# cgtuebingen/3D-RE-GEN

Hardware: NVIDIA H100
Metric: objects->mesh/sec (256^3 SDF, 50 DiT steps) (higher is better)
Workload: dtype f16

## Files before the change

3d-re-gen_b200/csrc/attn.cu:

```cuda
#include <cuda_fp16.h>
#include <math.h>

#include "r3g_internal.h"
#include "r3g_ptx.cuh"

namespace {

using namespace r3g;

constexpr int kD = 64;
constexpr int kWG = 3;
constexpr int kBQ = 64 * kWG;
constexpr int kBKV = 128;
constexpr int kStg = 3;
constexpr int kQBytes = 64 * kD * 2;
constexpr int kTileBytes = kBKV * kD * 2;
constexpr int kTilesBytes = kQBytes * kWG + 2 * kStg * kTileBytes;
constexpr int kSmemBytes = kTilesBytes + 1024 + 256;
constexpr int kThreads = 128 * kWG + 32;

struct AttnParams {
  __half* o;
  int64_t o_sb, o_sh, o_sl;
  int Lq, Lk;
  float scale_log2;
};

__device__ __forceinline__ float ex2(float x) {
  float y;
  asm("ex2.approx.ftz.f32 %0, %1;" : "=f"(y) : "f"(x));
  return y;
}

__global__ void __launch_bounds__(kThreads, 1)
attention_kernel(const __grid_constant__ CUtensorMap tmap_q, const __grid_constant__ CUtensorMap tmap_k,
                 const __grid_constant__ CUtensorMap tmap_v, const AttnParams p) {
  extern __shared__ uint8_t smem_raw[];
  uint8_t* smem = reinterpret_cast<uint8_t*>((reinterpret_cast<uintptr_t>(smem_raw) + 1023) & ~(uintptr_t)1023);
  uint8_t* sQ = smem;
  uint8_t* sK = sQ + kWG * kQBytes;
  uint8_t* sV = sK + kStg * kTileBytes;
  uint64_t* q_full = reinterpret_cast<uint64_t*>(smem + kTilesBytes);
  uint64_t* k_full = q_full + 1;
  uint64_t* v_full = k_full + kStg;
  uint64_t* k_empty = v_full + kStg;
  uint64_t* v_empty = k_empty + kStg;

  const int warp = threadIdx.x >> 5;
  const int lane = threadIdx.x & 31;
  const int q0 = blockIdx.x * kBQ;
  const int h = blockIdx.y, b = blockIdx.z;
  const int n_kv = (p.Lk + kBKV - 1) / kBKV;

  if (warp == 4 * kWG && lane == 0) {
    tma_prefetch_desc(&tmap_q);
    tma_prefetch_desc(&tmap_k);
    tma_prefetch_desc(&tmap_v);
    mbar_init(q_full, 1);
    for (int s = 0; s < kStg; ++s) {
      mbar_init(&k_full[s], 1);
      mbar_init(&v_full[s], 1);
      mbar_init(&k_empty[s], 128 * kWG);
      mbar_init(&v_empty[s], 128 * kWG);
    }
    fence_barrier_init();
  }
  __syncthreads();
  pdl_wait();

  if (warp == 4 * kWG) {
    if (lane == 0) {
      const int groups = min(kWG, (p.Lq - q0 + 63) / 64);
      mbar_expect_tx(q_full, groups * kQBytes);
      for (int g = 0; g < groups; ++g) tma_load_4d(sQ + g * kQBytes, &tmap_q, q_full, 0, q0 + 64 * g, h, b, kEvictFirst);
      for (int j = 0; j < n_kv; ++j) {
        const int st = j % kStg;
        const uint32_t ph = (j / kStg) & 1;
        mbar_wait(&k_empty[st], ph ^ 1);
        mbar_expect_tx(&k_full[st], kTileBytes);
        tma_load_4d(sK + st * kTileBytes, &tmap_k, &k_full[st], 0, j * kBKV, h, b, kEvictLast);
        mbar_wait(&v_empty[st], ph ^ 1);
        mbar_expect_tx(&v_full[st], kTileBytes);
        tma_load_4d(sV + st * kTileBytes, &tmap_v, &v_full[st], 0, j * kBKV, h, b, kEvictLast);
      }
    }
    return;
  }

  const int wg = warp >> 2;
  const int r0 = (warp & 3) * 16 + (lane >> 2);
  const int c0 = 2 * (lane & 3);
  const uint32_t aq = smem_u32(sQ + wg * kQBytes);
  float o[kD / 2];
#pragma unroll
  for (int i = 0; i < kD / 2; ++i) o[i] = 0.f;
  float m_run[2] = {-INFINITY, -INFINITY}, l_run[2] = {0.f, 0.f};
  mbar_wait(q_full, 0);
  for (int j = 0; j < n_kv; ++j) {
    const int st = j % kStg;
    const uint32_t ph = (j / kStg) & 1;
    float s[kBKV / 2];
    mbar_wait(&k_full[st], ph);
    const uint32_t ak = smem_u32(sK + st * kTileBytes);
    wgmma_fence();
#pragma unroll
    for (int k = 0; k < kD / 16; ++k)
      wgmma_m64n128k16_ss(s, gmma_desc_sw128(aq + k * 32, 1024, 16), gmma_desc_sw128(ak + k * 32, 1024, 16),
                          k ? 1u : 0u);
    wgmma_commit();
    wgmma_wait<0>();
    wgmma_reg_fence<kBKV / 2>(s);
    mbar_arrive(&k_empty[st]);

    const int valid = min(kBKV, p.Lk - j * kBKV);
    if (valid < kBKV) {
#pragma unroll
      for (int i = 0; i < kBKV / 2; ++i)
        if (8 * (i >> 2) + c0 + (i & 1) >= valid) s[i] = -INFINITY;
    }
    float mx[2] = {-INFINITY, -INFINITY};
#pragma unroll
    for (int i = 0; i < kBKV / 2; ++i) mx[(i >> 1) & 1] = fmaxf(mx[(i >> 1) & 1], s[i]);
    float alpha[2];
#pragma unroll
    for (int rr = 0; rr < 2; ++rr) {
      mx[rr] = fmaxf(mx[rr], __shfl_xor_sync(0xffffffffu, mx[rr], 1));
      mx[rr] = fmaxf(mx[rr], __shfl_xor_sync(0xffffffffu, mx[rr], 2));
      const float m_new = fmaxf(m_run[rr], mx[rr] * p.scale_log2);
      alpha[rr] = ex2(m_run[rr] - m_new);
      m_run[rr] = m_new;
      l_run[rr] *= alpha[rr];
    }
#pragma unroll
    for (int i = 0; i < kD / 2; ++i) o[i] *= alpha[(i >> 1) & 1];
    uint32_t pk[kBKV / 16][4];
#pragma unroll
    for (int i = 0; i < kBKV / 2; i += 2) {
      const int rr = (i >> 1) & 1;
      const float e0 = ex2(fmaf(s[i], p.scale_log2, -m_run[rr]));
      const float e1 = ex2(fmaf(s[i + 1], p.scale_log2, -m_run[rr]));
      l_run[rr] += e0 + e1;
      pk[i >> 3][(i >> 1) & 3] = pack_half2(e0, e1);
    }
    mbar_wait(&v_full[st], ph);
    const uint32_t av = smem_u32(sV + st * kTileBytes);
    wgmma_fence();
#pragma unroll
    for (int k = 0; k < kBKV / 16; ++k) wgmma_m64n64k16_rs_tb(o, pk[k], gmma_desc_sw128(av + k * 2048, 1024, 1024), 1u);
    wgmma_commit();
    wgmma_wait<0>();
    wgmma_reg_fence<kD / 2>(o);
    mbar_arrive(&v_empty[st]);
  }

  float inv_l[2];
#pragma unroll
  for (int rr = 0; rr < 2; ++rr) {
    float l = l_run[rr];
    l += __shfl_xor_sync(0xffffffffu, l, 1);
    l += __shfl_xor_sync(0xffffffffu, l, 2);
    inv_l[rr] = 1.f / l;
  }
#pragma unroll
  for (int rr = 0; rr < 2; ++rr) {
    const int qrow = q0 + wg * 64 + r0 + 8 * rr;
    if (qrow >= p.Lq) continue;
    __half* op = p.o + (int64_t)b * p.o_sb + (int64_t)h * p.o_sh + (int64_t)qrow * p.o_sl;
#pragma unroll
    for (int i = 2 * rr; i < kD / 2; i += 4)
      *reinterpret_cast<uint32_t*>(op + 8 * (i >> 2) + c0) = pack_half2(o[i] * inv_l[rr], o[i + 1] * inv_l[rr]);
  }
}

int make_qkv_map(r3g_ctx* ctx, CUtensorMap* m, const void* base, int64_t sb, int64_t sh, int64_t sl, int B, int H,
                 int L, int box_rows) {
  const uint64_t dims[4] = {(uint64_t)kD, (uint64_t)L, (uint64_t)H, (uint64_t)B};
  const uint64_t strides[4] = {2, (uint64_t)sl * 2, (uint64_t)sh * 2, (uint64_t)sb * 2};
  const uint32_t box[4] = {(uint32_t)kD, (uint32_t)box_rows, 1, 1};
  return r3g_make_tmap_f16(ctx, m, base, 4, dims, strides, box);
}

}

extern "C" int r3g_attention(r3g_ctx* ctx, const r3g_attention_args* a, void* stream) {
  r3g_device_guard guard(ctx);
  if (!ctx || !ctx->encode_tiled)
    return r3g_fail(ctx, R3G_E_CUDA, "attention: no CUDA device (there is no CPU fallback)");
  if (!a || !a->q || !a->k || !a->v || !a->o) return r3g_fail(ctx, R3G_E_INVALID, "attention: null argument");
  if (a->B < 1 || a->H < 1 || a->Lq < 1 || a->Lk < 1) return r3g_fail(ctx, R3G_E_INVALID, "attention: empty shape");
  if (a->o_sl % 8 || a->o_sh % 8 || a->o_sb % 8 || ((uintptr_t)a->o) % 16)
    return r3g_fail(ctx, R3G_E_INVALID, "attention: output strides must be multiples of 8 halfs");
  CUtensorMap mq, mk, mv;
  int rc;
  if ((rc = make_qkv_map(ctx, &mq, a->q, a->q_sb, a->q_sh, a->q_sl, a->B, a->H, a->Lq, 64))) return rc;
  if ((rc = make_qkv_map(ctx, &mk, a->k, a->k_sb, a->k_sh, a->k_sl, a->B, a->H, a->Lk, kBKV))) return rc;
  if ((rc = make_qkv_map(ctx, &mv, a->v, a->v_sb, a->v_sh, a->v_sl, a->B, a->H, a->Lk, kBKV))) return rc;
  AttnParams p;
  p.o = (__half*)a->o;
  p.o_sb = a->o_sb; p.o_sh = a->o_sh; p.o_sl = a->o_sl;
  p.Lq = a->Lq; p.Lk = a->Lk;
  p.scale_log2 = a->scale * 1.4426950408889634f;
  if (!(ctx->attr_done & R3G_ATTR_ATTENTION)) {
    R3G_CUDA_OK(ctx, cudaFuncSetAttribute(attention_kernel, cudaFuncAttributeMaxDynamicSharedMemorySize, kSmemBytes));
    R3G_CUDA_OK(ctx, cudaFuncSetAttribute(attention_kernel, cudaFuncAttributePreferredSharedMemoryCarveout, 100));
    ctx->attr_done |= R3G_ATTR_ATTENTION;
  }
  dim3 grid((a->Lq + kBQ - 1) / kBQ, a->H, a->B);
  R3G_CUDA_OK(ctx, r3g_launch_pdl(ctx, attention_kernel, grid, dim3(kThreads), kSmemBytes, (cudaStream_t)stream, mq, mk, mv, p));
  R3G_LAUNCH_OK(ctx);
  return R3G_OK;
}
```

3d-re-gen_b200/csrc/r3g_ptx.cuh:

```cuda
#pragma once
#include <cuda.h>
#include <cuda_fp16.h>
#include <cuda_runtime.h>
#include <stdint.h>

namespace r3g {

__device__ __forceinline__ uint32_t smem_u32(const void* p) {
  return static_cast<uint32_t>(__cvta_generic_to_shared(p));
}

__device__ __forceinline__ bool elect_one() {
  uint32_t pred = 0;
  asm volatile(
      "{\n\t.reg .pred P;\n\t"
      "elect.sync _|P, 0xffffffff;\n\t"
      "selp.u32 %0, 1, 0, P;\n\t}\n"
      : "=r"(pred));
  return pred != 0;
}

__device__ __forceinline__ void mbar_init(uint64_t* bar, uint32_t count) {
  asm volatile("mbarrier.init.shared::cta.b64 [%0], %1;\n" ::"r"(smem_u32(bar)), "r"(count));
}
__device__ __forceinline__ void pdl_wait() { asm volatile("griddepcontrol.wait;" ::: "memory"); }
__device__ __forceinline__ void pdl_trigger() { asm volatile("griddepcontrol.launch_dependents;" ::: "memory"); }

__device__ __forceinline__ void fence_barrier_init() {
  asm volatile("fence.mbarrier_init.release.cluster;\n" ::: "memory");
}
__device__ __forceinline__ void mbar_expect_tx(uint64_t* bar, uint32_t bytes) {
  asm volatile("mbarrier.arrive.expect_tx.shared::cta.b64 _, [%0], %1;\n" ::"r"(smem_u32(bar)), "r"(bytes)
               : "memory");
}
__device__ __forceinline__ void mbar_arrive(uint64_t* bar) {
  asm volatile("mbarrier.arrive.shared::cta.b64 _, [%0];\n" ::"r"(smem_u32(bar)) : "memory");
}
constexpr uint32_t kMbarSuspendHint = 0x989680u;
__device__ __forceinline__ bool mbar_try_wait(uint64_t* bar, uint32_t parity) {
  uint32_t ok;
  asm volatile(
      "{\n\t.reg .pred P;\n\t"
      "mbarrier.try_wait.parity.shared::cta.b64 P, [%1], %2, %3;\n\t"
      "selp.u32 %0, 1, 0, P;\n\t}\n"
      : "=r"(ok)
      : "r"(smem_u32(bar)), "r"(parity), "r"(kMbarSuspendHint)
      : "memory");
  return ok != 0;
}
__device__ __forceinline__ void mbar_wait(uint64_t* bar, uint32_t parity) {
  while (!mbar_try_wait(bar, parity)) {
  }
}

__device__ __forceinline__ void fence_proxy_async_smem() {
  asm volatile("fence.proxy.async.shared::cta;\n" ::: "memory");
}

__device__ __forceinline__ void named_bar_sync(uint32_t id, uint32_t count) {
  asm volatile("bar.sync %0, %1;\n" ::"r"(id), "r"(count) : "memory");
}

__device__ __forceinline__ void tma_prefetch_desc(const CUtensorMap* m) {
  asm volatile("prefetch.tensormap [%0];\n" ::"l"(reinterpret_cast<uint64_t>(m)) : "memory");
}
constexpr uint64_t kEvictNormal = 0x1000000000000000ull;
constexpr uint64_t kEvictFirst = 0x12F0000000000000ull;
constexpr uint64_t kEvictLast = 0x14F0000000000000ull;

__device__ __forceinline__ void tma_load_2d(void* smem_dst, const CUtensorMap* m, uint64_t* bar, int c0, int c1,
                                            uint64_t hint = kEvictNormal) {
  asm volatile(
      "cp.async.bulk.tensor.2d.shared::cluster.global.mbarrier::complete_tx::bytes.L2::cache_hint"
      " [%0], [%1, {%3, %4}], [%2], %5;\n" ::"r"(smem_u32(smem_dst)),
      "l"(reinterpret_cast<uint64_t>(m)), "r"(smem_u32(bar)), "r"(c0), "r"(c1), "l"(hint)
      : "memory");
}
__device__ __forceinline__ void tma_load_3d(void* smem_dst, const CUtensorMap* m, uint64_t* bar, int c0, int c1,
                                            int c2, uint64_t hint = kEvictNormal) {
  asm volatile(
      "cp.async.bulk.tensor.3d.shared::cluster.global.mbarrier::complete_tx::bytes.L2::cache_hint"
      " [%0], [%1, {%3, %4, %5}], [%2], %6;\n" ::"r"(smem_u32(smem_dst)),
      "l"(reinterpret_cast<uint64_t>(m)), "r"(smem_u32(bar)), "r"(c0), "r"(c1), "r"(c2), "l"(hint)
      : "memory");
}
__device__ __forceinline__ void tma_load_4d(void* smem_dst, const CUtensorMap* m, uint64_t* bar, int c0, int c1,
                                            int c2, int c3, uint64_t hint = kEvictNormal) {
  asm volatile(
      "cp.async.bulk.tensor.4d.shared::cluster.global.mbarrier::complete_tx::bytes.L2::cache_hint"
      " [%0], [%1, {%3, %4, %5, %6}], [%2], %7;\n" ::"r"(smem_u32(smem_dst)),
      "l"(reinterpret_cast<uint64_t>(m)), "r"(smem_u32(bar)), "r"(c0), "r"(c1), "r"(c2), "r"(c3), "l"(hint)
      : "memory");
}

__device__ __forceinline__ void wgmma_fence() { asm volatile("wgmma.fence.sync.aligned;\n" ::: "memory"); }
__device__ __forceinline__ void wgmma_commit() { asm volatile("wgmma.commit_group.sync.aligned;\n" ::: "memory"); }
template <int N>
__device__ __forceinline__ void wgmma_wait() {
  asm volatile("wgmma.wait_group.sync.aligned %0;\n" ::"n"(N) : "memory");
}
template <int N>
__device__ __forceinline__ void wgmma_reg_fence(float* d) {
#pragma unroll
  for (int i = 0; i < N; ++i) asm volatile("" : "+f"(d[i])::"memory");
}
__device__ __forceinline__ void wgmma_m64n128k16_ss(float* d, uint64_t desc_a, uint64_t desc_b, uint32_t accumulate) {
  asm volatile(
      "{\n\t.reg .pred p;\n\t"
      "setp.ne.b32 p, %66, 0;\n\t"
      "wgmma.mma_async.sync.aligned.m64n128k16.f32.f16.f16 "
      "{%0, %1, %2, %3, %4, %5, %6, %7, %8, %9, %10, %11, %12, %13, %14, %15, %16, %17, %18, %19, %20, %21, %22, %23, %24, %25, %26, %27, %28, %29, %30, %31, %32, %33, %34, %35, %36, %37, %38, %39, %40, %41, %42, %43, %44, %45, %46, %47, %48, %49, %50, %51, %52, %53, %54, %55, %56, %57, %58, %59, %60, %61, %62, %63}, "
      "%64, %65, p, 1, 1, 0, 0;\n\t}\n"
      : "+f"(d[0]), "+f"(d[1]), "+f"(d[2]), "+f"(d[3]), "+f"(d[4]), "+f"(d[5]), "+f"(d[6]), "+f"(d[7]), "+f"(d[8]), "+f"(d[9]), "+f"(d[10]), "+f"(d[11]), "+f"(d[12]), "+f"(d[13]), "+f"(d[14]), "+f"(d[15]), "+f"(d[16]), "+f"(d[17]), "+f"(d[18]), "+f"(d[19]), "+f"(d[20]), "+f"(d[21]), "+f"(d[22]), "+f"(d[23]), "+f"(d[24]), "+f"(d[25]), "+f"(d[26]), "+f"(d[27]), "+f"(d[28]), "+f"(d[29]), "+f"(d[30]), "+f"(d[31]), "+f"(d[32]), "+f"(d[33]), "+f"(d[34]), "+f"(d[35]), "+f"(d[36]), "+f"(d[37]), "+f"(d[38]), "+f"(d[39]), "+f"(d[40]), "+f"(d[41]), "+f"(d[42]), "+f"(d[43]), "+f"(d[44]), "+f"(d[45]), "+f"(d[46]), "+f"(d[47]), "+f"(d[48]), "+f"(d[49]), "+f"(d[50]), "+f"(d[51]), "+f"(d[52]), "+f"(d[53]), "+f"(d[54]), "+f"(d[55]), "+f"(d[56]), "+f"(d[57]), "+f"(d[58]), "+f"(d[59]), "+f"(d[60]), "+f"(d[61]), "+f"(d[62]), "+f"(d[63])
      : "l"(desc_a), "l"(desc_b), "r"(accumulate));
}
__device__ __forceinline__ void wgmma_m64n256k16_ss(float* d, uint64_t desc_a, uint64_t desc_b, uint32_t accumulate) {
  asm volatile(
      "{\n\t.reg .pred p;\n\t"
      "setp.ne.b32 p, %130, 0;\n\t"
      "wgmma.mma_async.sync.aligned.m64n256k16.f32.f16.f16 "
      "{%0, %1, %2, %3, %4, %5, %6, %7, %8, %9, %10, %11, %12, %13, %14, %15, %16, %17, %18, %19, %20, %21, %22, %23, %24, %25, %26, %27, %28, %29, %30, %31, %32, %33, %34, %35, %36, %37, %38, %39, %40, %41, %42, %43, %44, %45, %46, %47, %48, %49, %50, %51, %52, %53, %54, %55, %56, %57, %58, %59, %60, %61, %62, %63, %64, %65, %66, %67, %68, %69, %70, %71, %72, %73, %74, %75, %76, %77, %78, %79, %80, %81, %82, %83, %84, %85, %86, %87, %88, %89, %90, %91, %92, %93, %94, %95, %96, %97, %98, %99, %100, %101, %102, %103, %104, %105, %106, %107, %108, %109, %110, %111, %112, %113, %114, %115, %116, %117, %118, %119, %120, %121, %122, %123, %124, %125, %126, %127}, "
      "%128, %129, p, 1, 1, 0, 0;\n\t}\n"
      : "+f"(d[0]), "+f"(d[1]), "+f"(d[2]), "+f"(d[3]), "+f"(d[4]), "+f"(d[5]), "+f"(d[6]), "+f"(d[7]), "+f"(d[8]), "+f"(d[9]), "+f"(d[10]), "+f"(d[11]), "+f"(d[12]), "+f"(d[13]), "+f"(d[14]), "+f"(d[15]), "+f"(d[16]), "+f"(d[17]), "+f"(d[18]), "+f"(d[19]), "+f"(d[20]), "+f"(d[21]), "+f"(d[22]), "+f"(d[23]), "+f"(d[24]), "+f"(d[25]), "+f"(d[26]), "+f"(d[27]), "+f"(d[28]), "+f"(d[29]), "+f"(d[30]), "+f"(d[31]), "+f"(d[32]), "+f"(d[33]), "+f"(d[34]), "+f"(d[35]), "+f"(d[36]), "+f"(d[37]), "+f"(d[38]), "+f"(d[39]), "+f"(d[40]), "+f"(d[41]), "+f"(d[42]), "+f"(d[43]), "+f"(d[44]), "+f"(d[45]), "+f"(d[46]), "+f"(d[47]), "+f"(d[48]), "+f"(d[49]), "+f"(d[50]), "+f"(d[51]), "+f"(d[52]), "+f"(d[53]), "+f"(d[54]), "+f"(d[55]), "+f"(d[56]), "+f"(d[57]), "+f"(d[58]), "+f"(d[59]), "+f"(d[60]), "+f"(d[61]), "+f"(d[62]), "+f"(d[63]), "+f"(d[64]), "+f"(d[65]), "+f"(d[66]), "+f"(d[67]), "+f"(d[68]), "+f"(d[69]), "+f"(d[70]), "+f"(d[71]), "+f"(d[72]), "+f"(d[73]), "+f"(d[74]), "+f"(d[75]), "+f"(d[76]), "+f"(d[77]), "+f"(d[78]), "+f"(d[79]), "+f"(d[80]), "+f"(d[81]), "+f"(d[82]), "+f"(d[83]), "+f"(d[84]), "+f"(d[85]), "+f"(d[86]), "+f"(d[87]), "+f"(d[88]), "+f"(d[89]), "+f"(d[90]), "+f"(d[91]), "+f"(d[92]), "+f"(d[93]), "+f"(d[94]), "+f"(d[95]), "+f"(d[96]), "+f"(d[97]), "+f"(d[98]), "+f"(d[99]), "+f"(d[100]), "+f"(d[101]), "+f"(d[102]), "+f"(d[103]), "+f"(d[104]), "+f"(d[105]), "+f"(d[106]), "+f"(d[107]), "+f"(d[108]), "+f"(d[109]), "+f"(d[110]), "+f"(d[111]), "+f"(d[112]), "+f"(d[113]), "+f"(d[114]), "+f"(d[115]), "+f"(d[116]), "+f"(d[117]), "+f"(d[118]), "+f"(d[119]), "+f"(d[120]), "+f"(d[121]), "+f"(d[122]), "+f"(d[123]), "+f"(d[124]), "+f"(d[125]), "+f"(d[126]), "+f"(d[127])
      : "l"(desc_a), "l"(desc_b), "r"(accumulate));
}
__device__ __forceinline__ void wgmma_m64n64k16_rs_tb(float* d, const uint32_t* a, uint64_t desc_b, uint32_t accumulate) {
  asm volatile(
      "{\n\t.reg .pred p;\n\t"
      "setp.ne.b32 p, %37, 0;\n\t"
      "wgmma.mma_async.sync.aligned.m64n64k16.f32.f16.f16 "
      "{%0, %1, %2, %3, %4, %5, %6, %7, %8, %9, %10, %11, %12, %13, %14, %15, %16, %17, %18, %19, %20, %21, %22, %23, %24, %25, %26, %27, %28, %29, %30, %31}, "
      "{%32, %33, %34, %35}, %36, p, 1, 1, 1;\n\t}\n"
      : "+f"(d[0]), "+f"(d[1]), "+f"(d[2]), "+f"(d[3]), "+f"(d[4]), "+f"(d[5]), "+f"(d[6]), "+f"(d[7]), "+f"(d[8]), "+f"(d[9]), "+f"(d[10]), "+f"(d[11]), "+f"(d[12]), "+f"(d[13]), "+f"(d[14]), "+f"(d[15]), "+f"(d[16]), "+f"(d[17]), "+f"(d[18]), "+f"(d[19]), "+f"(d[20]), "+f"(d[21]), "+f"(d[22]), "+f"(d[23]), "+f"(d[24]), "+f"(d[25]), "+f"(d[26]), "+f"(d[27]), "+f"(d[28]), "+f"(d[29]), "+f"(d[30]), "+f"(d[31])
      : "r"(a[0]), "r"(a[1]), "r"(a[2]), "r"(a[3]), "l"(desc_b), "r"(accumulate));
}
__device__ __forceinline__ uint64_t f2_pack(float lo, float hi) {
  uint64_t r;
  asm("mov.b64 %0, {%1, %2};" : "=l"(r) : "f"(lo), "f"(hi));
  return r;
}
__device__ __forceinline__ void f2_unpack(uint64_t v, float& lo, float& hi) {
  asm("mov.b64 {%0, %1}, %2;" : "=f"(lo), "=f"(hi) : "l"(v));
}
__device__ __forceinline__ uint64_t f2_fma(uint64_t a, uint64_t b, uint64_t c) {
  float a0, a1, b0, b1, c0, c1;
  f2_unpack(a, a0, a1); f2_unpack(b, b0, b1); f2_unpack(c, c0, c1);
  return f2_pack(__fmaf_rn(a0, b0, c0), __fmaf_rn(a1, b1, c1));
}
__device__ __forceinline__ uint64_t f2_add(uint64_t a, uint64_t b) {
  float a0, a1, b0, b1;
  f2_unpack(a, a0, a1); f2_unpack(b, b0, b1);
  return f2_pack(__fadd_rn(a0, b0), __fadd_rn(a1, b1));
}
__device__ __forceinline__ uint64_t f2_mul(uint64_t a, uint64_t b) {
  float a0, a1, b0, b1;
  f2_unpack(a, a0, a1); f2_unpack(b, b0, b1);
  return f2_pack(__fmul_rn(a0, b0), __fmul_rn(a1, b1));
}

__device__ __forceinline__ uint64_t gmma_desc_sw128(uint32_t saddr, uint32_t sbo_bytes, uint32_t lbo_bytes) {
  uint64_t d = 0;
  d |= (uint64_t)((saddr & 0x3FFFF) >> 4);
  d |= (uint64_t)((lbo_bytes >> 4) & 0x3FFF) << 16;
  d |= (uint64_t)((sbo_bytes >> 4) & 0x3FFF) << 32;
  d |= (uint64_t)1 << 62;
  return d;
}

__device__ __forceinline__ uint32_t pack_half2(float a, float b) {
  __half2 h = __floats2half2_rn(a, b);
  return *reinterpret_cast<uint32_t*>(&h);
}

}
```

Measured before the change: 0.2704.

## Make attention kernel persistent with intra-warpgroup QK/PV overlap and ping-pong scheduling

Turns the attention kernel into a persistent kernel that loops over (q-tile, head, batch) tiles with a grid sized to the SM count, and double-buffers Q so the next tile's Q load overlaps the current one. Consumer warpgroups now issue the next QK GEMM before the current PV GEMM and run softmax while PV is in flight, FA3-style. Named barriers pass an MMA turn between warpgroups so tensor-core issue is serialized in a ping-pong. Producer warps give up registers through setmaxnreg so the consumers can hold more. The cost is more complex synchronization, extra shared memory for Q, and a full warpgroup assigned to the producer.

New measurement: 0.2766 (median of 6 runs). 1.02x the previous value.

```diff
diff --git a/3d-re-gen_b200/csrc/attn.cu b/3d-re-gen_b200/csrc/attn.cu
--- a/3d-re-gen_b200/csrc/attn.cu
+++ b/3d-re-gen_b200/csrc/attn.cu
@@ -13,17 +13,42 @@
 constexpr int kBQ = 64 * kWG;
 constexpr int kBKV = 128;
 constexpr int kStg = 3;
+constexpr int kQStg = 2;
 constexpr int kQBytes = 64 * kD * 2;
 constexpr int kTileBytes = kBKV * kD * 2;
-constexpr int kTilesBytes = kQBytes * kWG + 2 * kStg * kTileBytes;
+constexpr int kTilesBytes = kQStg * kWG * kQBytes + 2 * kStg * kTileBytes;
 constexpr int kSmemBytes = kTilesBytes + 1024 + 256;
-constexpr int kThreads = 128 * kWG + 32;
+constexpr int kThreads = 128 * (kWG + 1);
+constexpr int kProducerRegs = 24;
+constexpr int kConsumerRegs = 160;
+static_assert(128 * (kWG * kConsumerRegs + kProducerRegs) <= 65536, "register file");
 
 struct AttnParams {
   __half* o;
   int64_t o_sb, o_sh, o_sl;
   int Lq, Lk;
+  int H, n_qt, n_tiles;
   float scale_log2;
+};
+
+struct Tile {
+  int q0, h, b;
+};
+__device__ __forceinline__ Tile tile_at(int t, const AttnParams& p) {
+  const int bh = t / p.n_qt;
+  return {(t - bh * p.n_qt) * kBQ, bh % p.H, bh / p.H};
+}
+
+template <int kDepth>
+struct RingPos {
+  int st = 0;
+  uint32_t ph = 0;
+  __device__ __forceinline__ void next() {
+    if (++st == kDepth) {
+      st = 0;
+      ph ^= 1;
+    }
+  }
 };
 
 __device__ __forceinline__ float ex2(float x) {
@@ -31,6 +56,66 @@
   asm("ex2.approx.ftz.f32 %0, %1;" : "=f"(y) : "f"(x));
   return y;
 }
+
+__device__ __forceinline__ void reg_fence_a(uint32_t (&a)[kBKV / 16][4]) {
+#pragma unroll
+  for (int k = 0; k < kBKV / 16; ++k)
+#pragma unroll
+    for (int i = 0; i < 4; ++i) asm volatile("" : "+r"(a[k][i])::"memory");
+}
+
+__device__ __forceinline__ void issue_qk(float (&s)[kBKV / 2], uint32_t aq, uint32_t ak) {
+  wgmma_fence();
+#pragma unroll
+  for (int k = 0; k < kD / 16; ++k)
+    wgmma_m64n128k16_ss(s, gmma_desc_sw128(aq + k * 32, 1024, 16), gmma_desc_sw128(ak + k * 32, 1024, 16), k ? 1u : 0u);
+  wgmma_commit();
+}
+
+__device__ __forceinline__ void issue_pv(float (&o)[kD / 2], const uint32_t (&pk)[kBKV / 16][4], uint32_t av) {
+  wgmma_fence();
+#pragma unroll
+  for (int k = 0; k < kBKV / 16; ++k) wgmma_m64n64k16_rs_tb(o, pk[k], gmma_desc_sw128(av + k * 2048, 1024, 1024), 1u);
+  wgmma_commit();
+}
+
+__device__ __forceinline__ void softmax_tile(float (&s)[kBKV / 2], int valid, int c0, float scale_log2,
+                                             float (&m_run)[2], float (&l_run)[2], float (&alpha)[2]) {
+  if (valid < kBKV) {
+#pragma unroll
+    for (int i = 0; i < kBKV / 2; ++i)
+      if (8 * (i >> 2) + c0 + (i & 1) >= valid) s[i] = -INFINITY;
+  }
+  float mx[2] = {-INFINITY, -INFINITY};
+#pragma unroll
+  for (int i = 0; i < kBKV / 2; ++i) mx[(i >> 1) & 1] = fmaxf(mx[(i >> 1) & 1], s[i]);
+#pragma unroll
+  for (int rr = 0; rr < 2; ++rr) {
+    mx[rr] = fmaxf(mx[rr], __shfl_xor_sync(0xffffffffu, mx[rr], 1));
+    mx[rr] = fmaxf(mx[rr], __shfl_xor_sync(0xffffffffu, mx[rr], 2));
+    const float m_new = fmaxf(m_run[rr], mx[rr] * scale_log2);
+    alpha[rr] = ex2(m_run[rr] - m_new);
+    m_run[rr] = m_new;
+    l_run[rr] *= alpha[rr];
+  }
+#pragma unroll
+  for (int i = 0; i < kBKV / 2; i += 2) {
+    const int rr = (i >> 1) & 1;
+    const float e0 = ex2(fmaf(s[i], scale_log2, -m_run[rr]));
+    const float e1 = ex2(fmaf(s[i + 1], scale_log2, -m_run[rr]));
+    l_run[rr] += e0 + e1;
+    s[i] = e0;
+    s[i + 1] = e1;
+  }
+}
+
+__device__ __forceinline__ void pack_p(const float (&s)[kBKV / 2], uint32_t (&pk)[kBKV / 16][4]) {
+#pragma unroll
+  for (int i = 0; i < kBKV / 2; i += 2) pk[i >> 3][(i >> 1) & 3] = pack_half2(s[i], s[i + 1]);
+}
+
+__device__ __forceinline__ void mma_turn_wait() { named_bar_sync(1 + (threadIdx.x >> 7), 256); }
+__device__ __forceinline__ void mma_turn_pass() { named_bar_arrive(1 + ((threadIdx.x >> 7) + 1) % kWG, 256); }
 
 __global__ void __launch_bounds__(kThreads, 1)
 attention_kernel(const __grid_constant__ CUtensorMap tmap_q, const __grid_constant__ CUtensorMap tmap_k,
@@ -38,25 +123,27 @@
   extern __shared__ uint8_t smem_raw[];
   uint8_t* smem = reinterpret_cast<uint8_t*>((reinterpret_cast<uintptr_t>(smem_raw) + 1023) & ~(uintptr_t)1023);
   uint8_t* sQ = smem;
-  uint8_t* sK = sQ + kWG * kQBytes;
+  uint8_t* sK = sQ + kQStg * kWG * kQBytes;
   uint8_t* sV = sK + kStg * kTileBytes;
   uint64_t* q_full = reinterpret_cast<uint64_t*>(smem + kTilesBytes);
-  uint64_t* k_full = q_full + 1;
+  uint64_t* q_empty = q_full + kQStg;
+  uint64_t* k_full = q_empty + kQStg;
   uint64_t* v_full = k_full + kStg;
   uint64_t* k_empty = v_full + kStg;
   uint64_t* v_empty = k_empty + kStg;
 
   const int warp = threadIdx.x >> 5;
   const int lane = threadIdx.x & 31;
-  const int q0 = blockIdx.x * kBQ;
-  const int h = blockIdx.y, b = blockIdx.z;
   const int n_kv = (p.Lk + kBKV - 1) / kBKV;
 
   if (warp == 4 * kWG && lane == 0) {
     tma_prefetch_desc(&tmap_q);
     tma_prefetch_desc(&tmap_k);
     tma_prefetch_desc(&tmap_v);
-    mbar_init(q_full, 1);
+    for (int s = 0; s < kQStg; ++s) {
+      mbar_init(&q_full[s], 1);
+      mbar_init(&q_empty[s], 128 * kWG);
+    }
     for (int s = 0; s < kStg; ++s) {
       mbar_init(&k_full[s], 1);
       mbar_init(&v_full[s], 1);
@@ -68,108 +155,135 @@
   __syncthreads();
   pdl_wait();
 
-  if (warp == 4 * kWG) {
-    if (lane == 0) {
-      const int groups = min(kWG, (p.Lq - q0 + 63) / 64);
-      mbar_expect_tx(q_full, groups * kQBytes);
-      for (int g = 0; g < groups; ++g) tma_load_4d(sQ + g * kQBytes, &tmap_q, q_full, 0, q0 + 64 * g, h, b, kEvictFirst);
-      for (int j = 0; j < n_kv; ++j) {
-        const int st = j % kStg;
-        const uint32_t ph = (j / kStg) & 1;
-        mbar_wait(&k_empty[st], ph ^ 1);
-        mbar_expect_tx(&k_full[st], kTileBytes);
-        tma_load_4d(sK + st * kTileBytes, &tmap_k, &k_full[st], 0, j * kBKV, h, b, kEvictLast);
-        mbar_wait(&v_empty[st], ph ^ 1);
-        mbar_expect_tx(&v_full[st], kTileBytes);
-        tma_load_4d(sV + st * kTileBytes, &tmap_v, &v_full[st], 0, j * kBKV, h, b, kEvictLast);
+  if (warp >= 4 * kWG) {
+    setmaxnreg_dec<kProducerRegs>();
+    if (warp == 4 * kWG && lane == 0) {
+      RingPos<kQStg> qs;
+      RingPos<kStg> kv;
+      for (int t = blockIdx.x; t < p.n_tiles; t += gridDim.x) {
+        const Tile tl = tile_at(t, p);
+        const int groups = min(kWG, (p.Lq - tl.q0 + 63) / 64);
+        mbar_wait(&q_empty[qs.st], qs.ph ^ 1);
+        mbar_expect_tx(&q_full[qs.st], groups * kQBytes);
+        for (int g = 0; g < groups; ++g)
+          tma_load_4d(sQ + (qs.st * kWG + g) * kQBytes, &tmap_q, &q_full[qs.st], 0, tl.q0 + 64 * g, tl.h, tl.b,
+                      kEvictFirst);
+        qs.next();
+        for (int j = 0; j < n_kv; ++j, kv.next()) {
+          mbar_wait(&k_empty[kv.st], kv.ph ^ 1);
+          mbar_expect_tx(&k_full[kv.st], kTileBytes);
+          tma_load_4d(sK + kv.st * kTileBytes, &tmap_k, &k_full[kv.st], 0, j * kBKV, tl.h, tl.b, kEvictLast);
+          mbar_wait(&v_empty[kv.st], kv.ph ^ 1);
+          mbar_expect_tx(&v_full[kv.st], kTileBytes);
+          tma_load_4d(sV + kv.st * kTileBytes, &tmap_v, &v_full[kv.st], 0, j * kBKV, tl.h, tl.b, kEvictLast);
+        }
       }
     }
     return;
   }
 
+  setmaxnreg_inc<kConsumerRegs>();
   const int wg = warp >> 2;
-  const int r0 = (warp & 3) * 16 + (lane >> 2);
   const int c0 = 2 * (lane & 3);
-  const uint32_t aq = smem_u32(sQ + wg * kQBytes);
-  float o[kD / 2];
-#pragma unroll
-  for (int i = 0; i < kD / 2; ++i) o[i] = 0.f;
-  float m_run[2] = {-INFINITY, -INFINITY}, l_run[2] = {0.f, 0.f};
-  mbar_wait(q_full, 0);
-  for (int j = 0; j < n_kv; ++j) {
-    const int st = j % kStg;
-    const uint32_t ph = (j / kStg) & 1;
+  RingPos<kQStg> qs;
+  RingPos<kStg> kv;
+  if (wg == kWG - 1) mma_turn_pass();
+  for (int t = blockIdx.x; t < p.n_tiles; t += gridDim.x) {
+    mbar_wait(&q_full[qs.st], qs.ph);
+    if (tile_at(t, p).q0 + 64 * wg >= p.Lq) {
+      RingPos<kStg> kk = kv;
+      for (int j = 0; j <= n_kv; ++j) {
+        mma_turn_wait();
+        mma_turn_pass();
+        if (j < n_kv) {
+          mbar_wait(&k_full[kk.st], kk.ph);
+          mbar_arrive(&k_empty[kk.st]);
+          kk.next();
+        }
+        if (j > 0) {
+          mbar_wait(&v_full[kv.st], kv.ph);
+          mbar_arrive(&v_empty[kv.st]);
+          kv.next();
+        }
+      }
+      mbar_arrive(&q_empty[qs.st]);
+      qs.next();
+      continue;
+    }
+    const uint32_t aq = smem_u32(sQ + (qs.st * kWG + wg) * kQBytes);
+    float o[kD / 2];
+#pragma unroll
+    for (int i = 0; i < kD / 2; ++i) o[i] = 0.f;
+    float m_run[2] = {-INFINITY, -INFINITY}, l_run[2] = {0.f, 0.f}, alpha[2];
     float s[kBKV / 2];
-    mbar_wait(&k_full[st], ph);
-    const uint32_t ak = smem_u32(sK + st * kTileBytes);
-    wgmma_fence();
-#pragma unroll
-    for (int k = 0; k < kD / 16; ++k)
-      wgmma_m64n128k16_ss(s, gmma_desc_sw128(aq + k * 32, 1024, 16), gmma_desc_sw128(ak + k * 32, 1024, 16),
-                          k ? 1u : 0u);
-    wgmma_commit();
+    uint32_t pk[kBKV / 16][4];
+
+    mma_turn_wait();
+    mbar_wait(&k_full[kv.st], kv.ph);
+    issue_qk(s, aq, smem_u32(sK + kv.st * kTileBytes));
+    mma_turn_pass();
     wgmma_wait<0>();
     wgmma_reg_fence<kBKV / 2>(s);
-    mbar_arrive(&k_empty[st]);
-
-    const int valid = min(kBKV, p.Lk - j * kBKV);
-    if (valid < kBKV) {
-#pragma unroll
-      for (int i = 0; i < kBKV / 2; ++i)
-        if (8 * (i >> 2) + c0 + (i & 1) >= valid) s[i] = -INFINITY;
-    }
-    float mx[2] = {-INFINITY, -INFINITY};
-#pragma unroll
-    for (int i = 0; i < kBKV / 2; ++i) mx[(i >> 1) & 1] = fmaxf(mx[(i >> 1) & 1], s[i]);
-    float alpha[2];
-#pragma unroll
-    for (int rr = 0; rr < 2; ++rr) {
-      mx[rr] = fmaxf(mx[rr], __shfl_xor_sync(0xffffffffu, mx[rr], 1));
-      mx[rr] = fmaxf(mx[rr], __shfl_xor_sync(0xffffffffu, mx[rr], 2));
-      const float m_new = fmaxf(m_run[rr], mx[rr] * p.scale_log2);
-      alpha[rr] = ex2(m_run[rr] - m_new);
-      m_run[rr] = m_new;
-      l_run[rr] *= alpha[rr];
-    }
-#pragma unroll
-    for (int i = 0; i < kD / 2; ++i) o[i] *= alpha[(i >> 1) & 1];
-    uint32_t pk[kBKV / 16][4];
-#pragma unroll
-    for (int i = 0; i < kBKV / 2; i += 2) {
-      const int rr = (i >> 1) & 1;
-      const float e0 = ex2(fmaf(s[i], p.scale_log2, -m_run[rr]));
-      const float e1 = ex2(fmaf(s[i + 1], p.scale_log2, -m_run[rr]));
-      l_run[rr] += e0 + e1;
-      pk[i >> 3][(i >> 1) & 3] = pack_half2(e0, e1);
-    }
-    mbar_wait(&v_full[st], ph);
-    const uint32_t av = smem_u32(sV + st * kTileBytes);
-    wgmma_fence();
-#pragma unroll
-    for (int k = 0; k < kBKV / 16; ++k) wgmma_m64n64k16_rs_tb(o, pk[k], gmma_desc_sw128(av + k * 2048, 1024, 1024), 1u);
-    wgmma_commit();
+    mbar_arrive(&k_empty[kv.st]);
+    softmax_tile(s, min(kBKV, p.Lk), c0, p.scale_log2, m_run, l_run, alpha);
+    for (int j = 0;; ++j) {
+      wgmma_wait<0>();
+      wgmma_reg_fence<kD / 2>(o);
+      reg_fence_a(pk);
+      if (j > 0) {
+        mbar_arrive(&v_empty[kv.st]);
+        kv.next();
+      }
+#pragma unroll
+      for (int i = 0; i < kD / 2; ++i) o[i] *= alpha[(i >> 1) & 1];
+      pack_p(s, pk);
+      if (j + 1 == n_kv) break;
+      RingPos<kStg> nx = kv;
+      nx.next();
+      mma_turn_wait();
+      mbar_wait(&k_full[nx.st], nx.ph);
+      issue_qk(s, aq, smem_u32(sK + nx.st * kTileBytes));
+      mbar_wait(&v_full[kv.st], kv.ph);
+      issue_pv(o, pk, smem_u32(sV + kv.st * kTileBytes));
+      mma_turn_pass();
+      wgmma_wait<1>();
+      wgmma_reg_fence<kBKV / 2>(s);
+      mbar_arrive(&k_empty[nx.st]);
+      softmax_tile(s, min(kBKV, p.Lk - (j + 1) * kBKV), c0, p.scale_log2, m_run, l_run, alpha);
+    }
+    mma_turn_wait();
+    mbar_wait(&v_full[kv.st], kv.ph);
+    issue_pv(o, pk, smem_u32(sV + kv.st * kTileBytes));
+    mma_turn_pass();
     wgmma_wait<0>();
     wgmma_reg_fence<kD / 2>(o);
-    mbar_arrive(&v_empty[st]);
-  }
-
-  float inv_l[2];
-#pragma unroll
-  for (int rr = 0; rr < 2; ++rr) {
-    float l = l_run[rr];
-    l += __shfl_xor_sync(0xffffffffu, l, 1);
-    l += __shfl_xor_sync(0xffffffffu, l, 2);
-    inv_l[rr] = 1.f / l;
-  }
-#pragma unroll
-  for (int rr = 0; rr < 2; ++rr) {
-    const int qrow = q0 + wg * 64 + r0 + 8 * rr;
-    if (qrow >= p.Lq) continue;
-    __half* op = p.o + (int64_t)b * p.o_sb + (int64_t)h * p.o_sh + (int64_t)qrow * p.o_sl;
-#pragma unroll
-    for (int i = 2 * rr; i < kD / 2; i += 4)
-      *reinterpret_cast<uint32_t*>(op + 8 * (i >> 2) + c0) = pack_half2(o[i] * inv_l[rr], o[i + 1] * inv_l[rr]);
-  }
+    reg_fence_a(pk);
+    mbar_arrive(&v_empty[kv.st]);
+    kv.next();
+    mbar_arrive(&q_empty[qs.st]);
+    qs.next();
+
+    float inv_l[2];
+#pragma unroll
+    for (int rr = 0; rr < 2; ++rr) {
+      float l = l_run[rr];
+      l += __shfl_xor_sync(0xffffffffu, l, 1);
+      l += __shfl_xor_sync(0xffffffffu, l, 2);
+      inv_l[rr] = 1.f / l;
+    }
+    const Tile tl = tile_at(t, p);
+    const int r0 = ((threadIdx.x >> 1) & 48) + ((threadIdx.x & 31) >> 2);
+#pragma unroll
+    for (int rr = 0; rr < 2; ++rr) {
+      const int qrow = tl.q0 + wg * 64 + r0 + 8 * rr;
+      if (qrow >= p.Lq) continue;
+      __half* op = p.o + (int64_t)tl.b * p.o_sb + (int64_t)tl.h * p.o_sh + (int64_t)qrow * p.o_sl;
+#pragma unroll
+      for (int i = 2 * rr; i < kD / 2; i += 4)
+        *reinterpret_cast<uint32_t*>(op + 8 * (i >> 2) + c0) = pack_half2(o[i] * inv_l[rr], o[i + 1] * inv_l[rr]);
+    }
+  }
+  if (wg == 0) mma_turn_wait();
 }
 
 int make_qkv_map(r3g_ctx* ctx, CUtensorMap* m, const void* base, int64_t sb, int64_t sh, int64_t sl, int B, int H,
@@ -199,13 +313,18 @@
   p.o = (__half*)a->o;
   p.o_sb = a->o_sb; p.o_sh = a->o_sh; p.o_sl = a->o_sl;
   p.Lq = a->Lq; p.Lk = a->Lk;
+  p.H = a->H;
+  p.n_qt = (a->Lq + kBQ - 1) / kBQ;
+  const int64_t tiles = (int64_t)p.n_qt * a->H * a->B;
+  if (tiles > INT32_MAX) return r3g_fail(ctx, R3G_E_INVALID, "attention: too many query tiles");
+  p.n_tiles = (int)tiles;
   p.scale_log2 = a->scale * 1.4426950408889634f;
   if (!(ctx->attr_done & R3G_ATTR_ATTENTION)) {
     R3G_CUDA_OK(ctx, cudaFuncSetAttribute(attention_kernel, cudaFuncAttributeMaxDynamicSharedMemorySize, kSmemBytes));
     R3G_CUDA_OK(ctx, cudaFuncSetAttribute(attention_kernel, cudaFuncAttributePreferredSharedMemoryCarveout, 100));
     ctx->attr_done |= R3G_ATTR_ATTENTION;
   }
-  dim3 grid((a->Lq + kBQ - 1) / kBQ, a->H, a->B);
+  const dim3 grid((unsigned)(tiles < ctx->num_sms ? tiles : ctx->num_sms));
   R3G_CUDA_OK(ctx, r3g_launch_pdl(ctx, attention_kernel, grid, dim3(kThreads), kSmemBytes, (cudaStream_t)stream, mq, mk, mv, p));
   R3G_LAUNCH_OK(ctx);
   return R3G_OK;
diff --git a/3d-re-gen_b200/csrc/r3g_ptx.cuh b/3d-re-gen_b200/csrc/r3g_ptx.cuh
--- a/3d-re-gen_b200/csrc/r3g_ptx.cuh
+++ b/3d-re-gen_b200/csrc/r3g_ptx.cuh
@@ -53,12 +53,20 @@
   }
 }
 
+template <int N>
+__device__ __forceinline__ void setmaxnreg_dec() { asm volatile("setmaxnreg.dec.sync.aligned.u32 %0;\n" ::"n"(N)); }
+template <int N>
+__device__ __forceinline__ void setmaxnreg_inc() { asm volatile("setmaxnreg.inc.sync.aligned.u32 %0;\n" ::"n"(N)); }
+
 __device__ __forceinline__ void fence_proxy_async_smem() {
   asm volatile("fence.proxy.async.shared::cta;\n" ::: "memory");
 }
 
 __device__ __forceinline__ void named_bar_sync(uint32_t id, uint32_t count) {
   asm volatile("bar.sync %0, %1;\n" ::"r"(id), "r"(count) : "memory");
+}
+__device__ __forceinline__ void named_bar_arrive(uint32_t id, uint32_t count) {
+  asm volatile("bar.arrive %0, %1;\n" ::"r"(id), "r"(count) : "memory");
 }
 
 __device__ __forceinline__ void tma_prefetch_desc(const CUtensorMap* m) {
```

## Software-pipeline attention QK and PV wgmma with producer/consumer register reallocation

Applied to the files above, without the earlier changes.

Restructures the attention consumer loop so the QK^T wgmma for tile j is issued together with the PV wgmma for tile j-1. Softmax on the new scores then runs while the PV matmul is in flight, hiding tensor-core latency behind exp work. The producer is widened to a full warpgroup that calls setmaxnreg to give up registers, so consumer warpgroups can raise their limit to 160. Empty barriers now count only the active warpgroups, and idle ones exit early. The extra live registers (scores plus the packed P from the previous tile) add spill risk, and the ordering of waits and barriers is harder to get right.

New measurement: 0.2682 before, 0.2702 after (median of 6 runs). Within noise of the previous version (+0.7%).

```diff
diff --git a/3d-re-gen_b200/csrc/attn.cu b/3d-re-gen_b200/csrc/attn.cu
--- a/3d-re-gen_b200/csrc/attn.cu
+++ b/3d-re-gen_b200/csrc/attn.cu
@@ -17,7 +17,9 @@
 constexpr int kTileBytes = kBKV * kD * 2;
 constexpr int kTilesBytes = kQBytes * kWG + 2 * kStg * kTileBytes;
 constexpr int kSmemBytes = kTilesBytes + 1024 + 256;
-constexpr int kThreads = 128 * kWG + 32;
+constexpr int kThreads = 128 * (kWG + 1);
+constexpr uint32_t kProducerRegs = 24, kConsumerRegs = 160;
+static_assert(128 * kProducerRegs + 128 * kWG * kConsumerRegs <= 65536, "register split exceeds the register file");
 
 struct AttnParams {
   __half* o;
@@ -30,6 +32,87 @@
   float y;
   asm("ex2.approx.ftz.f32 %0, %1;" : "=f"(y) : "f"(x));
   return y;
+}
+
+__device__ __forceinline__ void issue_qk(float (&s)[kBKV / 2], uint32_t aq, uint32_t ak) {
+#pragma unroll
+  for (int k = 0; k < kD / 16; ++k)
+    wgmma_m64n128k16_ss(s, gmma_desc_sw128(aq + k * 32, 1024, 16), gmma_desc_sw128(ak + k * 32, 1024, 16), k ? 1u : 0u);
+}
+
+__device__ __forceinline__ void issue_pv(float (&o)[kD / 2], const uint32_t (&pk)[kBKV / 16][4], uint32_t av) {
+#pragma unroll
+  for (int k = 0; k < kBKV / 16; ++k) wgmma_m64n64k16_rs_tb(o, pk[k], gmma_desc_sw128(av + k * 2048, 1024, 1024), 1u);
+}
+
+template <bool kMask>
+__device__ __forceinline__ void softmax_tile(float (&s)[kBKV / 2], float (&m_run)[2], float (&l_run)[2],
+                                             float (&alpha)[2], int valid, int c0, float scale_log2) {
+  if (kMask) {
+#pragma unroll
+    for (int i = 0; i < kBKV / 2; ++i) s[i] = 8 * (i >> 2) + c0 + (i & 1) >= valid ? -INFINITY : s[i];
+  }
+  float mx[2] = {-INFINITY, -INFINITY};
+#pragma unroll
+  for (int i = 0; i < kBKV / 2; ++i) mx[(i >> 1) & 1] = fmaxf(mx[(i >> 1) & 1], s[i]);
+#pragma unroll
+  for (int rr = 0; rr < 2; ++rr) {
+    mx[rr] = fmaxf(mx[rr], __shfl_xor_sync(0xffffffffu, mx[rr], 1));
+    mx[rr] = fmaxf(mx[rr], __shfl_xor_sync(0xffffffffu, mx[rr], 2));
+    const float m_new = fmaxf(m_run[rr], mx[rr] * scale_log2);
+    alpha[rr] = ex2(m_run[rr] - m_new);
+    m_run[rr] = m_new;
+    l_run[rr] *= alpha[rr];
+  }
+#pragma unroll
+  for (int i = 0; i < kBKV / 2; i += 2) {
+    const int rr = (i >> 1) & 1;
+    const float e0 = ex2(fmaf(s[i], scale_log2, -m_run[rr]));
+    const float e1 = ex2(fmaf(s[i + 1], scale_log2, -m_run[rr]));
+    l_run[rr] += e0 + e1;
+    s[i] = e0;
+    s[i + 1] = e1;
+  }
+}
+
+__device__ __forceinline__ void pack_p(uint32_t (&pk)[kBKV / 16][4], const float (&s)[kBKV / 2]) {
+#pragma unroll
+  for (int i = 0; i < kBKV / 2; i += 2) pk[i >> 3][(i >> 1) & 3] = pack_half2(s[i], s[i + 1]);
+}
+
+__device__ __forceinline__ void pin_before_wait(uint32_t sink, float v) {
+  asm volatile("st.shared.f32 [%0], %1;\n" ::"r"(sink), "f"(v) : "memory");
+}
+
+template <bool kMask>
+__device__ __forceinline__ void pipelined_tile(int j, int valid, float (&o)[kD / 2], uint32_t (&pk)[kBKV / 16][4],
+                                               float (&m_run)[2], float (&l_run)[2], float (&alpha)[2], uint32_t aq,
+                                               int c0, uint8_t* sK, uint8_t* sV, uint64_t* k_full, uint64_t* v_full,
+                                               uint64_t* k_empty, uint64_t* v_empty, uint32_t sink,
+                                               float scale_log2) {
+  const int st = j % kStg, pst = (j - 1) % kStg;
+  const uint32_t ph = (j / kStg) & 1, pph = ((j - 1) / kStg) & 1;
+  float s[kBKV / 2];
+  mbar_wait(&k_full[st], ph);
+  wgmma_fence();
+  issue_qk(s, aq, smem_u32(sK + st * kTileBytes));
+  wgmma_commit();
+#pragma unroll
+  for (int i = 0; i < kD / 2; ++i) o[i] *= alpha[(i >> 1) & 1];
+  mbar_wait(&v_full[pst], pph);
+  wgmma_fence();
+  issue_pv(o, pk, smem_u32(sV + pst * kTileBytes));
+  wgmma_commit();
+  wgmma_wait<1>();
+  wgmma_reg_fence<kBKV / 2>(s);
+  mbar_arrive(&k_empty[st]);
+  softmax_tile<kMask>(s, m_run, l_run, alpha, valid, c0, scale_log2);
+  pin_before_wait(sink, l_run[0] + l_run[1]);
+  wgmma_wait<0>();
+  wgmma_reg_fence<kD / 2>(o);
+  wgmma_reg_fence_u32<kBKV / 8>(&pk[0][0]);
+  mbar_arrive(&v_empty[pst]);
+  pack_p(pk, s);
 }
 
 __global__ void __launch_bounds__(kThreads, 1)
@@ -45,12 +128,14 @@
   uint64_t* v_full = k_full + kStg;
   uint64_t* k_empty = v_full + kStg;
   uint64_t* v_empty = k_empty + kStg;
+  const uint32_t sink = smem_u32(v_empty + kStg);
 
   const int warp = threadIdx.x >> 5;
   const int lane = threadIdx.x & 31;
   const int q0 = blockIdx.x * kBQ;
   const int h = blockIdx.y, b = blockIdx.z;
   const int n_kv = (p.Lk + kBKV - 1) / kBKV;
+  const int groups = min(kWG, (p.Lq - q0 + 63) / 64);
 
   if (warp == 4 * kWG && lane == 0) {
     tma_prefetch_desc(&tmap_q);
@@ -60,17 +145,17 @@
     for (int s = 0; s < kStg; ++s) {
       mbar_init(&k_full[s], 1);
       mbar_init(&v_full[s], 1);
-      mbar_init(&k_empty[s], 128 * kWG);
-      mbar_init(&v_empty[s], 128 * kWG);
+      mbar_init(&k_empty[s], 128 * groups);
+      mbar_init(&v_empty[s], 128 * groups);
     }
     fence_barrier_init();
   }
   __syncthreads();
   pdl_wait();
 
-  if (warp == 4 * kWG) {
-    if (lane == 0) {
-      const int groups = min(kWG, (p.Lq - q0 + 63) / 64);
+  if (warp >= 4 * kWG) {
+    setmaxnreg_dec<kProducerRegs>();
+    if (warp == 4 * kWG && lane == 0) {
       mbar_expect_tx(q_full, groups * kQBytes);
       for (int g = 0; g < groups; ++g) tma_load_4d(sQ + g * kQBytes, &tmap_q, q_full, 0, q0 + 64 * g, h, b, kEvictFirst);
       for (int j = 0; j < n_kv; ++j) {
@@ -87,66 +172,43 @@
     return;
   }
 
+  setmaxnreg_inc<kConsumerRegs>();
   const int wg = warp >> 2;
+  if (wg >= groups) return;
   const int r0 = (warp & 3) * 16 + (lane >> 2);
   const int c0 = 2 * (lane & 3);
   const uint32_t aq = smem_u32(sQ + wg * kQBytes);
   float o[kD / 2];
 #pragma unroll
   for (int i = 0; i < kD / 2; ++i) o[i] = 0.f;
-  float m_run[2] = {-INFINITY, -INFINITY}, l_run[2] = {0.f, 0.f};
+  float m_run[2] = {-INFINITY, -INFINITY}, l_run[2] = {0.f, 0.f}, alpha[2];
+  uint32_t pk[kBKV / 16][4];
   mbar_wait(q_full, 0);
-  for (int j = 0; j < n_kv; ++j) {
-    const int st = j % kStg;
-    const uint32_t ph = (j / kStg) & 1;
+  {
     float s[kBKV / 2];
-    mbar_wait(&k_full[st], ph);
-    const uint32_t ak = smem_u32(sK + st * kTileBytes);
+    mbar_wait(&k_full[0], 0);
     wgmma_fence();
-#pragma unroll
-    for (int k = 0; k < kD / 16; ++k)
-      wgmma_m64n128k16_ss(s, gmma_desc_sw128(aq + k * 32, 1024, 16), gmma_desc_sw128(ak + k * 32, 1024, 16),
-                          k ? 1u : 0u);
+    issue_qk(s, aq, smem_u32(sK));
     wgmma_commit();
     wgmma_wait<0>();
     wgmma_reg_fence<kBKV / 2>(s);
-    mbar_arrive(&k_empty[st]);
-
-    const int valid = min(kBKV, p.Lk - j * kBKV);
-    if (valid < kBKV) {
-#pragma unroll
-      for (int i = 0; i < kBKV / 2; ++i)
-        if (8 * (i >> 2) + c0 + (i & 1) >= valid) s[i] = -INFINITY;
-    }
-    float mx[2] = {-INFINITY, -INFINITY};
-#pragma unroll
-    for (int i = 0; i < kBKV / 2; ++i) mx[(i >> 1) & 1] = fmaxf(mx[(i >> 1) & 1], s[i]);
-    float alpha[2];
-#pragma unroll
-    for (int rr = 0; rr < 2; ++rr) {
-      mx[rr] = fmaxf(mx[rr], __shfl_xor_sync(0xffffffffu, mx[rr], 1));
-      mx[rr] = fmaxf(mx[rr], __shfl_xor_sync(0xffffffffu, mx[rr], 2));
-      const float m_new = fmaxf(m_run[rr], mx[rr] * p.scale_log2);
-      alpha[rr] = ex2(m_run[rr] - m_new);
-      m_run[rr] = m_new;
-      l_run[rr] *= alpha[rr];
-    }
+    mbar_arrive(&k_empty[0]);
+    softmax_tile<true>(s, m_run, l_run, alpha, min(kBKV, p.Lk), c0, p.scale_log2);
+    pack_p(pk, s);
+  }
+  for (int j = 1; j < n_kv - 1; ++j)
+    pipelined_tile<false>(j, kBKV, o, pk, m_run, l_run, alpha, aq, c0, sK, sV, k_full, v_full, k_empty, v_empty, sink,
+                          p.scale_log2);
+  if (n_kv > 1)
+    pipelined_tile<true>(n_kv - 1, p.Lk - (n_kv - 1) * kBKV, o, pk, m_run, l_run, alpha, aq, c0, sK, sV, k_full,
+                         v_full, k_empty, v_empty, sink, p.scale_log2);
+  {
+    const int st = (n_kv - 1) % kStg;
 #pragma unroll
     for (int i = 0; i < kD / 2; ++i) o[i] *= alpha[(i >> 1) & 1];
-    uint32_t pk[kBKV / 16][4];
-#pragma unroll
-    for (int i = 0; i < kBKV / 2; i += 2) {
-      const int rr = (i >> 1) & 1;
-      const float e0 = ex2(fmaf(s[i], p.scale_log2, -m_run[rr]));
-      const float e1 = ex2(fmaf(s[i + 1], p.scale_log2, -m_run[rr]));
-      l_run[rr] += e0 + e1;
-      pk[i >> 3][(i >> 1) & 3] = pack_half2(e0, e1);
-    }
-    mbar_wait(&v_full[st], ph);
-    const uint32_t av = smem_u32(sV + st * kTileBytes);
+    mbar_wait(&v_full[st], ((n_kv - 1) / kStg) & 1);
     wgmma_fence();
-#pragma unroll
-    for (int k = 0; k < kBKV / 16; ++k) wgmma_m64n64k16_rs_tb(o, pk[k], gmma_desc_sw128(av + k * 2048, 1024, 1024), 1u);
+    issue_pv(o, pk, smem_u32(sV + st * kTileBytes));
     wgmma_commit();
     wgmma_wait<0>();
     wgmma_reg_fence<kD / 2>(o);
diff --git a/3d-re-gen_b200/csrc/r3g_ptx.cuh b/3d-re-gen_b200/csrc/r3g_ptx.cuh
--- a/3d-re-gen_b200/csrc/r3g_ptx.cuh
+++ b/3d-re-gen_b200/csrc/r3g_ptx.cuh
@@ -61,6 +61,15 @@
   asm volatile("bar.sync %0, %1;\n" ::"r"(id), "r"(count) : "memory");
 }
 
+template <uint32_t N>
+__device__ __forceinline__ void setmaxnreg_dec() {
+  asm volatile("setmaxnreg.dec.sync.aligned.u32 %0;\n" ::"n"(N));
+}
+template <uint32_t N>
+__device__ __forceinline__ void setmaxnreg_inc() {
+  asm volatile("setmaxnreg.inc.sync.aligned.u32 %0;\n" ::"n"(N));
+}
+
 __device__ __forceinline__ void tma_prefetch_desc(const CUtensorMap* m) {
   asm volatile("prefetch.tensormap [%0];\n" ::"l"(reinterpret_cast<uint64_t>(m)) : "memory");
 }
@@ -103,6 +112,11 @@
 __device__ __forceinline__ void wgmma_reg_fence(float* d) {
 #pragma unroll
   for (int i = 0; i < N; ++i) asm volatile("" : "+f"(d[i])::"memory");
+}
+template <int N>
+__device__ __forceinline__ void wgmma_reg_fence_u32(uint32_t* a) {
+#pragma unroll
+  for (int i = 0; i < N; ++i) asm volatile("" : "+r"(a[i])::"memory");
 }
 __device__ __forceinline__ void wgmma_m64n128k16_ss(float* d, uint64_t desc_a, uint64_t desc_b, uint32_t accumulate) {
   asm volatile(
```
